# edin-dal/sdqlpy

Hardware: AMD Instinct MI355X
Metric: tpch_q1_q3_q5_sf10_rows_per_sec (higher is better)
Workload: dtype f64; 1 GPU; TPCH Q1+Q3+Q5 SF=10 per GPU (BASELINE metric: Q1/Q3/Q5 at SF=10; q1 = configs[1], q3 = configs[2]); partitioning=none

## Files before the change

### sdqlpy_amd/csrc/sdqh_hip.hip

```cpp
#include <hip/hip_runtime.h>

#include <algorithm>
#include <atomic>
#include <chrono>
#include <cmath>
#include <cstdio>
#include <cstdlib>
#include <cstring>
#include <string>
#include <thread>
#include <type_traits>
#include <map>
#include <vector>

#include "sdqh_host.hpp"

using namespace sdqh_host;

static int ensure_index(sdqh_ctx* ctx, sdqh_table* tb);

namespace sdqh_host {

int fail(sdqh_ctx* ctx, int code, const std::string& msg) {
    if (ctx) ctx->err = msg;
// ... 626 lines not shown
    else if (n == "delta8" && (value == 0 || value == 1)) ctx->opt_delta8 = (int)value;
    else if (n == "word_pairs" && (value == 0 || value == 1)) ctx->opt_word_pairs = (int)value;
    else if (n == "coarse_kb" && value >= 0 && value <= 96) ctx->opt_coarse_kb = (int)value;
    else if (n == "lookup_pipeline" && value >= -1 && value <= 1) ctx->opt_lookup_pipeline = (int)value;
    else if (n == "probe_pipeline" && value >= 0 && value <= 1) ctx->opt_probe_pipeline = (int)value;
    else if (n == "lookup_debug") ctx->opt_lookup_debug = (int)value;
    else if (n == "fuse_small" && value >= 0 && value <= 1) ctx->opt_fuse_small = (int)value;
    else if (n == "lds_key_set" && value >= 0 && value <= 1) ctx->opt_lds_key_set = (int)value;
    else if (n == "fill_ahead" && value >= 0 && value <= 1) { ctx->opt_fill_ahead = (int)value; for (auto& b : ctx->pool) b.nhabits = 0; }
    else if (n == "str_rows" && (value == 0 || value == 32 || value == 64)) ctx->opt_str_rows = (int)value;
    else if (n == "rank_increasing" && value >= 0 && value <= 1) ctx->opt_rank_increasing = (int)value;
    else if (n == "feature_min_rows" && value >= 0) ctx->opt_feature_min_rows = value;
    else if (n == "narrow" && value >= 0 && value <= 1) ctx->opt_narrow = (int)value;
    else if (n == "tight" && value >= 0 && value <= 1) ctx->opt_tight = (int)value;
    else if (n == "spin_sync" && value >= 0 && value <= 1) ctx->opt_spin_sync = (int)value;
    else if (n == "vstage" && value >= 0 && value <= 1) ctx->opt_vstage = (int)value;
    else if (n == "side_streams" && value >= 0 && value <= 1) ctx->opt_side_streams = (int)value;
    else if (n == "side_priority" && value >= 0 && value <= 1) ctx->opt_side_priority = (int)value;
    else if (n == "copy_kernel" && value >= 0 && value <= 4096) ctx->opt_copy_kernel = (int)value;
    else if (n == "copy_nt" && value >= 0 && value <= 1) ctx->opt_copy_nt = (int)value;
    else if (n == "x_waves" && value >= 0 && value <= 256) ctx->opt_x_waves = (int)value;
    else if (n == "window" && value >= 0 && value <= 1) ctx->opt_window = (int)value;
    else if (n == "lane_int" && value >= 0 && value <= 1) ctx->opt_lane_int = (int)value;
    else if (n == "row_index" && value >= 0 && value <= 1) ctx->opt_row_index = (int)value;
    else if (n == "lane_resident" && value >= 1 && value <= 4) ctx->opt_lane_resident = (int)value;
    else if (n == "async_result" && value >= 0 && value <= 1) ctx->opt_async_result = (int)value;
    else if (n == "stage_pipeline" && value >= 0 && value <= 1) ctx->opt_stage_pipeline = (int)value;
    else if (n == "span_index" && value >= 0 && value <= 1) ctx->opt_span_index = (int)value;
    else if (n == "dense_increasing" && value >= 0 && value <= 1) ctx->opt_dense_increasing = (int)value;
    else if (n == "packed_slots" && (value == 0 || value == 1)) ctx->opt_packed_slots = (int)value;
    else if (n == "grouped_index" && (value == 0 || value == 1)) ctx->opt_grouped_index = (int)value;
    else if (n == "grouped_pairs" && (value == 0 || value == 1)) ctx->opt_grouped_pairs = (int)value;
    else if (n == "index_inline" && (value == 0 || value == 1)) ctx->opt_index_inline = (int)value;
    else if (n == "groupby_regs" && (value == 0 || value == 4 || value == 8)) ctx->opt_groupby_regs = (int)value;
    else if (n == "hash_filter" && (value == 0 || value == 1)) ctx->opt_hash_filter = (int)value;
    else if (n == "pack_ordered" && (value == 0 || value == 1)) ctx->opt_pack_ordered = (int)value;
    else if (n == "pool_trim" && value == 1) {
        if (ctx->compile_only) return SDQH_OK;
        if (ctx->capturing) return fail(ctx, SDQH_ERR_UNSUPPORTED, "set_option: pool_trim inside a recording");
        (void)hipSetDevice(ctx->device);
        if (hipStreamSynchronize(ctx->stream) != hipSuccess) { (void)hipGetLastError(); return fail(ctx, SDQH_ERR_DEVICE, "pool_trim: the stream failed"); }
        for (auto& b : ctx->pool) if (b.free && b.ptr && !b.graph_owner) { (void)hipFree(b.ptr); b.ptr = nullptr; }
        ctx->pool.erase(std::remove_if(ctx->pool.begin(), ctx->pool.end(), [](const PoolBlock& b) { return b.ptr == nullptr; }), ctx->pool.end());
    }
    else return fail(ctx, SDQH_ERR_INVALID, "set_option: unknown option or value out of range: " + n);
    return SDQH_OK;
}

int sdqh_memory_stats(sdqh_ctx* ctx, int64_t* out, int n) {
    if (!ctx || !out || n < 4) return fail(ctx, SDQH_ERR_INVALID, "memory_stats: bad arguments");
    int64_t used = 0, cached = 0, graphs = 0, blocks = 0;
    for (const auto& b : ctx->pool) {
        if (!b.ptr) continue;
        ++blocks;
        if (b.graph_owner) graphs += (int64_t)b.size;
        if (b.free && !b.graph_owner) cached += (int64_t)b.size; else used += (int64_t)b.size;
    }
    out[0] = used; out[1] = cached; out[2] = graphs; out[3] = blocks;
    return SDQH_OK;
}

static int new_column(sdqh_ctx* ctx, int64_t nrows, int dtype, int width, sdqh_column** out) {
    if (!ctx || !out || nrows < 0) return fail(ctx, SDQH_ERR_INVALID, "column: bad arguments");
    if (dtype != SDQH_I64 && dtype != SDQH_F64 && dtype != SDQH_STR) return fail(ctx, SDQH_ERR_INVALID, "column: bad dtype");
    if (dtype == SDQH_STR && width < 1) return fail(ctx, SDQH_ERR_INVALID, "column: STR needs width >= 1");
    sdqh_column* c = new sdqh_column();
// ... 1272 lines not shown
        if (want_bm && ctx->opt_direct_index) { tb->nwords = lin_rb ? (lin_bits + 31) / 32 : ((uint64_t)(hi - lo) + 32) / 32; tb->bm = static_cast<uint32_t*>(table_alloc(ctx, tb, tb->nwords * 4 + 64)); }
        if (!tb->hdr || !flags || (tb->nwords && !tb->bm)) rc = fail(ctx, SDQH_ERR_NOMEM, "build: out of device memory");
    }
    uint32_t* grp_first = nullptr;
    const size_t grp_cells = grouped ? (size_t)(hi - lo) + 1 : 0;
    if (!rc && grouped && tb->bm) grp_first = static_cast<uint32_t*>(table_alloc(ctx, tb, grp_cells * 4 + 64));
    if (!rc) {
        tb->dev.hdr = tb->hdr; tb->dev.shits = tb->stage.shits; tb->dev.sacc = tb->stage.sacc; tb->dev.acc_stride = tb->stage.acc_stride;
        if (grp_first) {
            tb->stage.grp_first = grp_first;
            tb->dev.grp_first = grp_first; tb->dev.grp_key = tb->stage.key; tb->dev.grp_kstride = 1; tb->dev.grp_seg_rows = tb->stage.seg_rows;
            if (npayload >= 1 && ctx->opt_grouped_pairs) {
                int64_t* kp = static_cast<int64_t*>(table_alloc(ctx, tb, ((size_t)nrows + 8) * 16 + 64));
                if (kp) { tb->stage.grp_kp = kp; tb->dev.grp_key = kp; tb->dev.grp_kstride = 2; }
            } tb->dev.grp_cap = nrows + 1;
        }
        const int shift = (nkey == 2 && !(tb->bm && lin_rb)) ? 32 : 0;
        tb->dev.bm = tb->bm; tb->dev.bm_lo = lo; tb->dev.bm_hi = hi; tb->dev.bitmap_only = 0; tb->dev.bm_shift = shift;
        for (int p = 0; p < npayload; ++p) tb->dev.pay[p] = tb->stage.pay[p];
        tb->stage.bm = tb->bm; tb->stage.bm_lo = lo; tb->stage.bm_hi = hi; tb->stage.hdr = tb->hdr; tb->stage.bm_shift = shift;
        if (tb->bm && lin_rb) { tb->dev.lin_rb = tb->stage.lin_rb = lin_rb; tb->dev.lin_b0 = tb->stage.lin_b0 = lin_b0; }
        const unsigned seg_grid = (unsigned)((tb->stage.nseg + TPB / WAVE - 1) / (TPB / WAVE));
        FillList fl; fl.add(tb->hdr, sizeof(TableHeader), 0); fl.add(flags, 8, 0); if (tb->bm) fl.add(tb->bm, tb->nwords * 4, 0); prefill_refs(ctx, tb, &fl);
        if (grp_first) fl.add(grp_first, grp_cells * 4, 0xFF);
        DevFill pre; std::memset(&pre, 0, sizeof(pre));
        prune_clean(ctx, &fl);
        if (seg_grid == 1 && ctx->opt_fuse_small && fl.most <= ((uint64_t)1 << 20) && fl.f.n <= FILL_MAX) pre = fl.pre(); else launch_fill(ctx, fl);
        DevIndexInline ix; std::memset(&ix, 0, sizeof(ix));
        if (seg_grid == 1 && ctx->opt_fuse_small && ctx->opt_index_inline && tb->bm && shift == 0 && tb->refs_prefilled && (tb->nwords + RANK_BLOCK_WORDS - 1) / RANK_BLOCK_WORDS == 1) {
            uint32_t* wprefix = static_cast<uint32_t*>(table_alloc(ctx, tb, tb->nwords * 4 + 64));
            if (wprefix) {
                tb->dev.wprefix = wprefix;
                ix.t = tb->dev; ix.wprefix = wprefix; ix.span = tb->span; ix.nwords = tb->nwords; ix.on = 1;
            }
        }
        hipError_t e;
        with_scan_filter(f, [&](auto FC) {
            using FCT = decltype(FC);
            if constexpr (std::is_same_v<FCT, FCfg<1, 0, 0, 0>> || std::is_same_v<FCT, FCfg<0, 0, 0, 0>>) {
                const bool eager0 = nlookups > 0 && lookups[0].key[0].kind == SDQH_SRC_COLUMN && lookups[0].key[0].col->dtype == SDQH_I64;
                if (ctx->opt_narrow && nrows >= ctx->opt_feature_min_rows && (eager0 || f.ni == 1)) {
                    const int32_t* nkey0 = eager0 ? static_cast<const int32_t*>(ensure_narrow(ctx, const_cast<sdqh_column*>(lookups[0].key[0].col))) : nullptr;
                    const int32_t* npred0 = f.ni == 1 ? static_cast<const int32_t*>(ensure_narrow(ctx, const_cast<sdqh_column*>(filter->ipred[0].col))) : nullptr;
                    if ((!eager0 || nkey0) && (f.ni != 1 || npred0)) {
                        auto kern = k_build_lookup<FCT, true>;
                        LAUNCH(ctx, "k_build_lookup", kern, seg_grid, f, L, spec, tb->stage, nrows, flags, nkey0, npred0, pre, ix);
                        return SDQH_OK;
                    }
                }
            }
            auto kern = k_build_lookup<FCT>;
            LAUNCH(ctx, "k_build_lookup", kern, seg_grid, f, L, spec, tb->stage, nrows, flags, static_cast<const int32_t*>(nullptr), static_cast<const int32_t*>(nullptr), pre, ix);
            return SDQH_OK;
        });
        if (ix.on) { if (tb->span) tb->dev.dense_arr = tb->span; tb->index_built = true; }
        call_end(ctx);
        e = hipGetLastError();
        if (e != hipSuccess) rc = fail(ctx, SDQH_ERR_DEVICE, std::string("build launch: ") + hipGetErrorString(e));
        auto packs = [&](const sdqh_source& src) {
            if (src.kind != SDQH_SRC_COLUMN || !src.col || src.col->dtype != SDQH_I64) return false;
            sdqh_column* c = const_cast<sdqh_column*>(src.col);
            return ensure_minmax(ctx, c) == SDQH_OK && c->nrows > 0 && c->mn >= 0 && c->mx <= 0xFFFFFFFFll;
        };
        bool proven = composite;
        if (composite && !rc) {
            if (nkey == 2) proven = proven && packs(key[0]) && packs(key[1]);
            for (int l = 0; l < nlookups && proven; ++l) if (lookups[l].nkey == 2) proven = packs(lookups[l].key[0]) && packs(lookups[l].key[1]);
        }
        if (!rc && composite && !proven) {
            e = hipMemcpyAsync(ctx->result_host, flags, 4, hipMemcpyDeviceToHost, ctx->stream);
            if (e != hipSuccess) rc = fail(ctx, SDQH_ERR_DEVICE, hipGetErrorString(e));
            if (!rc) rc = sync_stream(ctx);
            if (!rc && (*static_cast<const int*>(ctx->result_host) & 2)) rc = fail(ctx, SDQH_ERR_UNSUPPORTED, "build: composite key part outside [0, 2^32)");
        }
    }
    if (rc) { table_release(ctx, tb); delete tb; return rc; }
    *out = tb;
    return SDQH_OK;
}

static int lookup_aggregate_launch(sdqh_ctx* ctx, int64_t nrows, const sdqh_filter* filter, int nlookups, const sdqh_lookup* lookups,
                                   int nkeys, const sdqh_source* keys, int tuple_shape, const sdqh_source* operands, void* block, bool device_block) {
    (void)hipSetDevice(ctx->device);
    const int nops = tuple_nops(tuple_shape), nv = tuple_nv(tuple_shape);
    if (nops < 0) return fail(ctx, SDQH_ERR_UNSUPPORTED, "unknown tuple shape");
// ... 556 lines not shown
```

### sdqlpy_amd/csrc/sdqh_host.hpp

```cpp
#pragma once
#include <hip/hip_runtime.h>

#include <atomic>
#include <map>
#include <string>
#include <vector>

#include "sdqh.h"
#include "sdqh_kernels.hpp"

namespace sdqh_host {

struct FillHabit { size_t off, bytes; int byte; bool clean; };
struct PoolBlock {
    void* ptr; size_t size; bool free;
    FillHabit habits[4] = {};
    int nhabits = 0;
    uint64_t alloc_seq = 0;
    bool fill_use = false;
    const void* graph_owner = nullptr;
};
struct ProfEntry { const char* name; hipEvent_t e0, e1; double ms; int64_t model_bytes; };

constexpr size_t STAGING_BYTES = 32u << 20;
// ... 43 lines not shown
    int opt_probe_chunk = 1;
    int opt_resident_stream = 2;
    int opt_probe_unroll = PROBE_UNROLL;
    int opt_stage_batch = STAGE_BATCH;
    int opt_stage_eager = 1;
    int nested = 0;
    int opt_stage_eager_pay = 0;
    int opt_stage_waves_per_cu = 12;
    int opt_direct_index = 1;
    int opt_packed_slots = 1;
    int opt_lookup_pipeline = -1;
    int opt_lookup_debug = 0;
    size_t rd_clean_ff = 0; int64_t rd_clean_zero_off = -1;
    int opt_fill_ahead = 1;
    uint64_t launch_seq = 0;
    int opt_lds_key_set = 1;
    int opt_fuse_small = 1;
    int opt_str_rows = 0;
    int opt_rank_increasing = 1;
    int64_t opt_feature_min_rows = 1 << 20;
    bool in_groupby_key = false;
    int opt_vstage = 1;
    int opt_tight = 1;
    hipStream_t side[2] = {nullptr, nullptr};
    hipEvent_t side_ev[4] = {nullptr, nullptr, nullptr, nullptr};
    int opt_side_streams = 1;
    int opt_side_priority = 1;
    int opt_copy_kernel = 0;
    int opt_copy_nt = 1;
    int opt_row_index = 1;
    int opt_grouped_index = 1;
    int opt_grouped_pairs = 1;
    int opt_index_inline = 1;
    int opt_lane_int = 1;
    int opt_lane_resident = 2;
    int opt_window = 0;
    int opt_x_driven = 64;
    int opt_word_pairs = 0;
    int opt_delta8 = 1;
    int opt_x_waves = 0;
    void* rs_dev[2] = {nullptr, nullptr}; size_t rs_bytes[2] = {0, 0};
    hipEvent_t rs_copied[2] = {nullptr, nullptr}; bool rs_used[2] = {false, false};
    int rs_cur = 0; bool rs_pending = false;
    hipEvent_t rs_ready = nullptr;
    volatile uint32_t* sync_flag = nullptr; uint32_t sync_seq = 0; int opt_spin_sync = 1;
    int opt_async_result = 1;
    int opt_narrow = 1;
    int opt_stage_pipeline = 0;
    int opt_span_index = 1;
    int opt_dense_increasing = 1;
    int opt_probe_pipeline = 0;
    const void* coarse_stat_col = nullptr; uint64_t* coarse_stat = nullptr;
    unsigned long long* coarse_count_dev = nullptr; uint64_t coarse_stat_bits_pending = 0; int coarse_skipped = 0; int64_t coarse_stat_build_rows = -1;
    int opt_coarse_kb = 64;
    int opt_row_pack = 1;
    struct RowPack { std::vector<const void*> cols; int64_t nrows; int k; void* data; const void* order_col = nullptr; void* key32 = nullptr;
                     void* lb = nullptr; int64_t key_lo = 0, key_hi = -1; };
    std::vector<RowPack> packs;
    int opt_pack_ordered = 1;
    int opt_hash_filter = 1;
    int opt_cluster_list = 1;
    int opt_cluster_pack = 1;
    int opt_groupby_regs = 0;
    const void* g4_hint[SDQH_MAX_GROUPKEYS] = {nullptr, nullptr};
};

// ... 136 lines not shown
```

### sdqlpy_amd/csrc/sdqh_kernels.hpp

```cpp
#pragma once
#ifndef __HIPCC_RTC__
#include <hip/hip_runtime.h>
#include <stdint.h>
#endif
#include "sdqh.h"

#if defined(__HIPCC_RTC__) || defined(SDQH_DECLS_ONLY)
#define SDQH_KERNEL template <int SDQH_RTC_UNUSED = 0> __global__
#else
#define SDQH_KERNEL __global__
#endif

namespace sdqh {

constexpr int TPB = 256;
constexpr int WAVE = 64;
constexpr int ROWS_PER_LOAD = 2;
#ifndef SDQH_UNROLL
#define SDQH_UNROLL 2
#endif
#ifndef SDQH_NT_LOADS
#define SDQH_NT_LOADS 1
#endif
#ifndef SDQH_TILE_CHUNK
// ... 63 lines not shown
    const int64_t* grp_key;
    int64_t grp_kstride;
    int64_t grp_seg_rows, grp_cap;
    const unsigned long long* wpair;
    uint32_t* hf;
};
constexpr int HF_SHIFT = 2;
constexpr uint32_t HF_POS_MASK = 0x07FFFFFFu;
constexpr uint64_t HF_MAX_CAP = 1ull << 22;
constexpr uint32_t HF_DEGENERATE = 127u;
__device__ __forceinline__ uint32_t hf_mask_of(uint64_t cap_mask) { return cap_mask + 1 > HF_MAX_CAP ? HF_DEGENERATE : (uint32_t)(((cap_mask + 1) << HF_SHIFT) - 1); }
__device__ __forceinline__ uint32_t hf_raw(int64_t key);
__device__ __forceinline__ uint32_t hf_code(uint32_t raw, uint32_t mask) { return (raw & mask) | (raw & ~HF_POS_MASK); }
__device__ __forceinline__ uint32_t hf_bits(uint32_t code) { return (1u << (code & 31u)) | (1u << (code >> 27)); }
__device__ __forceinline__ bool hf_test(uint32_t word, uint32_t code) { return ((word >> (code & 31u)) & (word >> (code >> 27)) & 1u) != 0u; }

constexpr int FILL_MAX = 6;
struct DevFill { void* p[FILL_MAX]; uint64_t bytes[FILL_MAX]; uint32_t word[FILL_MAX]; int32_t n, _pad; };
constexpr int FILL_BIG = 32;
struct DevFillBig { void* p[FILL_BIG]; uint64_t bytes[FILL_BIG]; uint32_t word[FILL_BIG]; int32_t n, _pad; };
__device__ __forceinline__ void fill_in_block(const DevFill& f) {
#pragma unroll
    for (int r = 0; r < FILL_MAX; ++r) {
        if (r >= f.n) break;
        const uint32_t w = f.word[r];
        const uint64_t n16 = f.bytes[r] / 16, n4 = f.bytes[r] / 4;
        uint4* p16 = static_cast<uint4*>(f.p[r]);
        for (uint64_t i = threadIdx.x; i < n16; i += blockDim.x) p16[i] = make_uint4(w, w, w, w);
        uint32_t* p4 = static_cast<uint32_t*>(f.p[r]);
        for (uint64_t i = n16 * 4 + threadIdx.x; i < n4; i += blockDim.x) p4[i] = w;
    }
}

__device__ __forceinline__ int64_t slot_key(const DevTable& t, uint64_t h) { return t.slots ? t.slots[h * 4] : t.keys[h]; }
__device__ __forceinline__ uint32_t slot_row(const DevTable& t, uint64_t h) { return t.slots ? (uint32_t)t.slots[h * 4 + 3] : t.rowref[h]; }

template <class T>
__device__ __forceinline__ bool bm_locate(const T& t, int64_t key, uint64_t& off) {
    const int64_t rb = t.lin_rb;
    const int64_t v = (t.bm_shift || rb) ? (int64_t)((uint64_t)key >> 32) : key;
    if (v < t.bm_lo || v > t.bm_hi) return false;
    off = (uint64_t)(v - t.bm_lo);
    if (rb) {
        const int64_t b = (int64_t)((uint64_t)key & 0xFFFFFFFFull) - t.lin_b0;
        if (b < 0 || b >= rb) return false;
        off = off * (uint64_t)rb + (uint64_t)b;
    }
    return true;
}

template <int SHAPE> struct TupleTraits;
template <> struct TupleTraits<SDQH_TUPLE_A>          { static constexpr int NOPS = 1, NV = 1; };
template <> struct TupleTraits<SDQH_TUPLE_AB>         { static constexpr int NOPS = 2, NV = 1; };
template <> struct TupleTraits<SDQH_TUPLE_A_1MB>      { static constexpr int NOPS = 2, NV = 1; };
template <> struct TupleTraits<SDQH_TUPLE_PRICING>    { static constexpr int NOPS = 4, NV = 4; };
template <> struct TupleTraits<SDQH_TUPLE_A_1MB_M_CD> { static constexpr int NOPS = 4, NV = 1; };
template <> struct TupleTraits<SDQH_TUPLE_COUNT>      { static constexpr int NOPS = 0, NV = 0; };

template <int SHAPE>
__device__ __forceinline__ void tuple_eval(const double (&x)[4], double (&o)[4]) {
    if constexpr (SHAPE == SDQH_TUPLE_A) { o[0] = x[0]; }
    else if constexpr (SHAPE == SDQH_TUPLE_AB) { o[0] = x[0] * x[1]; }
    else if constexpr (SHAPE == SDQH_TUPLE_A_1MB) { o[0] = x[0] * (1.0 - x[1]); }
    else if constexpr (SHAPE == SDQH_TUPLE_PRICING) {
        double dp = x[1] * (1.0 - x[2]);
        o[0] = x[0]; o[1] = x[1]; o[2] = dp; o[3] = dp * (1.0 + x[3]);
// ... 1236 lines not shown
    }
    int t = s - 1;
    while (t > 0 && st.seg_count[t] == 0) --t;
    WordExc e;
    e.key0 = f.key; e.pos0 = f.pos; e.n0 = n_below; e._pad = 0;
    e.pos_prev = (uint32_t)((int64_t)t * st.seg_rows + (int64_t)st.seg_count[t] - (int64_t)n_below);
    exc[s] = e;
    st.wrow[w0] = ROW_INDEX_EXC | (uint32_t)s;
}
__device__ __forceinline__ bool direct_has_dups(const TableHeader* hdr) { return hdr->staged != hdr->distinct; }
SDQH_KERNEL __launch_bounds__(TPB) void k_fill_refs(DevStage st, DevTable t) {
    if (!direct_has_dups(t.hdr)) return;
    const uint64_t n = t.hdr->distinct;
    for (uint64_t i = (uint64_t)blockIdx.x * TPB + threadIdx.x; i < n; i += (uint64_t)gridDim.x * TPB) t.dense_ref[i] = NO_ROW;
}
__device__ __forceinline__ void insert_direct_body(const DevStage& st, const DevTable& t, uint32_t* __restrict__ span) {
    const int seg = blockIdx.x * (TPB / WAVE) + threadIdx.x / WAVE;
    const bool dups = direct_has_dups(t.hdr);
    if (blockIdx.x == 0 && threadIdx.x == 0) t.hdr->has_dups = dups ? 1u : 0u;
    if (seg >= st.nseg) return;
    const int64_t base = (int64_t)seg * st.seg_rows;
    const uint32_t count = st.seg_count[seg];
    for (uint32_t i = lane_id(); i < count; i += WAVE) {
        const int64_t idx = base + i;
        const int64_t pos = table_find(t, st.key[idx], 0);
        if (pos < 0) continue;
        if (dups) atomicMin(&t.dense_ref[pos], (uint32_t)idx); else t.dense_ref[pos] = (uint32_t)idx;
        if (span) { uint32_t* cell = span + (st.key[idx] - t.bm_lo); if (dups) atomicMin(cell, (uint32_t)idx); else *cell = (uint32_t)idx; }
    }
}
SDQH_KERNEL __launch_bounds__(TPB) void k_insert_direct(DevStage st, DevTable t, uint32_t* __restrict__ span) { insert_direct_body(st, t, span); }
SDQH_KERNEL __launch_bounds__(TPB) void k_index_small(const uint32_t* __restrict__ bm, uint64_t nwords, uint32_t* __restrict__ wprefix, DevStage st, DevTable t, uint32_t* __restrict__ span) {
    rank_words_body(bm, nwords, wprefix, st.seg_count, st.nseg, t.hdr);
    __threadfence();
    __syncthreads();
    insert_direct_body(st, t, span);
}
SDQH_KERNEL __launch_bounds__(TPB) void k_index_medium(const uint32_t* __restrict__ bm, uint32_t nwords, uint32_t* __restrict__ wprefix, DevStage st, DevTable t, uint32_t* __restrict__ span) {
    __shared__ uint32_t s_word[RANK_BLOCK_WORDS], s_pre[RANK_BLOCK_WORDS];
    __shared__ uint32_t s_wave[TPB / WAVE];
    __shared__ uint32_t s_staged;
    constexpr int PER = RANK_BLOCK_WORDS / TPB;
    const int lane = lane_id(), w = threadIdx.x / WAVE;
    for (int i = threadIdx.x; i < RANK_BLOCK_WORDS; i += TPB) s_word[i] = (uint32_t)i < nwords ? bm[i] : 0u;
    if (threadIdx.x == 0) s_staged = 0u;
    __syncthreads();
    uint32_t mine = 0;
#pragma unroll
    for (int j = 0; j < PER; ++j) mine += (uint32_t)__popc(s_word[threadIdx.x * PER + j]);
    uint32_t incl = mine;
#pragma unroll
    for (int off = 1; off < WAVE; off <<= 1) { const uint32_t v = __shfl_up(incl, off, WAVE); if (lane >= off) incl += v; }
    if (lane == WAVE - 1) s_wave[w] = incl;
    uint32_t stg = 0;
    for (int i = threadIdx.x; i < st.nseg; i += TPB) stg += st.seg_count[i];
#pragma unroll
    for (int off = WAVE / 2; off > 0; off >>= 1) stg += __shfl_down(stg, off, WAVE);
    if (lane == 0 && stg) atomicAdd(&s_staged, stg);
    __syncthreads();
    uint32_t before = 0, total = 0;
#pragma unroll
    for (int i = 0; i < TPB / WAVE; ++i) { if (i < w) before += s_wave[i]; total += s_wave[i]; }
    uint32_t run = before + incl - mine;
#pragma unroll
    for (int j = 0; j < PER; ++j) { s_pre[threadIdx.x * PER + j] = run; run += (uint32_t)__popc(s_word[threadIdx.x * PER + j]); }
    __syncthreads();
    const uint32_t staged = s_staged;
    const bool dups = staged != total;
// ... 757 lines not shown
    if (!t.bm) return true;
    if (L.l[0].nkey == 2 && t.bm_shift == 0) return true;
    if (part0 < t.bm_lo || part0 > t.bm_hi) return false;
    const uint64_t off = (uint64_t)(part0 - t.bm_lo);
    return (t.bm[off >> 5] >> (off & 31)) & 1u;
}

__device__ __forceinline__ bool first_lookup_none(const DevLookups& L) {
    const DevTable& t = L.l[0].table;
    return !t.bm || (L.l[0].nkey == 2 && t.bm_shift == 0);
}
__device__ __forceinline__ uint32_t first_lookup_word(const DevLookups& L, int64_t part0) {
    const DevTable& t = L.l[0].table;
    const bool in = part0 >= t.bm_lo && part0 <= t.bm_hi;
    const uint64_t off = in ? (uint64_t)(part0 - t.bm_lo) : 0;
    return t.bm[off >> 5];
}
__device__ __forceinline__ bool first_lookup_bit(const DevLookups& L, int64_t part0, uint32_t word) {
    const DevTable& t = L.l[0].table;
    const bool in = part0 >= t.bm_lo && part0 <= t.bm_hi;
    return in && ((word >> ((uint64_t)(part0 - t.bm_lo) & 31)) & 1u);
}

constexpr int BUILD_LB = 4;
constexpr int LOOKUP_PU = 2;
constexpr int LBQ_CAP = 64 + BUILD_LB * 128;

struct DevBuildSpec {
    int32_t nkey, npay;
    DevSource key[2];
    DevSource pay[SDQH_MAX_PAYLOAD];
};

struct DevIndexInline { DevTable t; uint32_t* wprefix; uint32_t* span; uint64_t nwords; int32_t on, _pad; };

template <class FC, bool NW>
__device__ __forceinline__ void build_lookup_segment(const DevFilter& f, const DevLookups& L, const DevBuildSpec& spec, const DevStage& st, int64_t nrows, int* __restrict__ flags,
                                                     const int32_t* __restrict__ nkey0, const int32_t* __restrict__ npred0, int32_t* q_row, const int seg) {
    const int64_t* skey0 = NW ? reinterpret_cast<const int64_t*>(nkey0) : L.l[0].key[0].col;
    const int64_t begin = (int64_t)seg * st.seg_rows;
    int64_t end = begin + st.seg_rows; if (end > nrows) end = nrows;
    const int lane = lane_id();
    const uint64_t lt = lanemask_lt();
    constexpr int64_t BATCH_ROWS = WAVE * ROWS_PER_LOAD;
    const bool eager0 = L.n > 0 && L.l[0].key[0].kind == SDQH_SRC_COLUMN;
    DevProbes none; none.n = 0;
    const uint64_t nomask[SDQH_MAX_PROBE] = {0, 0};
    int64_t out = begin;
    int qn = 0;
    bool bad = false;
    auto drain = [&](int first, int count) {
        bool keep = false; int64_t key = 0; int64_t pay[MAX_STAGE_COLS] = {0, 0, 0, 0, 0};
        if (lane < count) {
            const int64_t r = begin + (int64_t)q_row[first + lane];
            uint32_t ent[SDQH_MAX_LOOKUP] = {0, 0, 0};
            const PackRow nopack{};
            const int h = run_lookups(L, r, ent, nopack);
            if (h < 0) bad = true;
            if (h > 0) {
                const int64_t p0 = source_value(spec.key[0], L, r, ent, nopack);
                const int64_t p1 = spec.nkey == 2 ? source_value(spec.key[1], L, r, ent, nopack) : 0;
                if (pack_parts(spec.nkey, p0, p1, key)) bad = true;
                else {
                    keep = true;
#pragma unroll
                    for (int q = 0; q < SDQH_MAX_PAYLOAD; ++q) if (q < spec.npay) pay[q] = source_value(spec.pay[q], L, r, ent, nopack);
                }
// ... 59 lines not shown
            enqueue(r, p1b[0][0], p1b[0][1]);
            b += BATCH_ROWS;
        }
        int head = 0;
        while (qn - head >= WAVE || (last && qn > head)) {
            const int n = qn - head >= WAVE ? WAVE : qn - head;
            drain(head, n);
            head += n;
        }
        if (last) break;
        if (head) {
            const int left = qn - head;
            int32_t keepv = 0;
            if (lane < left) keepv = q_row[head + lane];
            if (lane < left) q_row[lane] = keepv;
            qn = left;
        }
    }
    if (lane == 0) {
        st.seg_count[seg] = (uint32_t)(out - begin);
        stage_end_segment(st, seg, begin, out - begin);
        if (st.grp_first && seg == 0) st.hdr->has_dups = 1u;
    }
    if (__ballot(bad) && lane == 0) atomicOr(flags, 2);
}

template <class FC, bool NW = false>
__global__ __launch_bounds__(TPB) void k_build_lookup(DevFilter f, DevLookups L, DevBuildSpec spec, DevStage st, int64_t nrows, int* __restrict__ flags,
                                                      const int32_t* __restrict__ nkey0, const int32_t* __restrict__ npred0, DevFill pre, DevIndexInline ix) {
    if (pre.n) { fill_in_block(pre); __syncthreads(); }
    __shared__ int32_t s_row[TPB / WAVE][LBQ_CAP];
    const int seg = blockIdx.x * (TPB / WAVE) + threadIdx.x / WAVE;
    if (seg < st.nseg) build_lookup_segment<FC, NW>(f, L, spec, st, nrows, flags, nkey0, npred0, s_row[threadIdx.x / WAVE], seg);
    if (ix.on) {
        __threadfence();
        __syncthreads();
        rank_words_body(st.bm, ix.nwords, ix.wprefix, st.seg_count, st.nseg, st.hdr);
        __threadfence();
        __syncthreads();
        insert_direct_body(st, ix.t, ix.span);
    }
}

struct DevPackCols { const int64_t* col[MAX_PACK]; int32_t ncols, k; };
SDQH_KERNEL __launch_bounds__(TPB) void k_interleave(DevPackCols c, int64_t nrows, int64_t* __restrict__ out) {
    for (int64_t r = (int64_t)blockIdx.x * TPB + threadIdx.x; r < nrows; r += (int64_t)gridDim.x * TPB) {
        int64_t v[MAX_PACK];
#pragma unroll
        for (int j = 0; j < MAX_PACK; ++j) v[j] = j < c.ncols ? c.col[j][r] : 0;
#pragma unroll
        for (int j = 0; j < MAX_PACK; ++j) if (j < c.k) out[r * c.k + j] = v[j];
    }
}

constexpr int LG_SLOTS = 2 * SDQH_MAX_LOOKUP_GROUPS;

struct DevAggSpec {
    int32_t nkeys, shape;
    DevSource key[SDQH_MAX_GROUPKEYS];
    DevSource op[4];
};

__device__ __forceinline__ int group_slot(unsigned long long* keys, unsigned long long key, bool global) {
    int h = (int)(mix64(key) & (LG_SLOTS - 1));
#pragma unroll 1
    for (int i = 0; i < LG_SLOTS; ++i) {
        unsigned long long cur = global ? __hip_atomic_load(&keys[h], __ATOMIC_RELAXED, __HIP_MEMORY_SCOPE_AGENT) : keys[h];
        if (cur == EMPTY_GROUP) cur = atomicCAS(&keys[h], (unsigned long long)EMPTY_GROUP, key);
        if (cur == EMPTY_GROUP || cur == key) return h;
        h = (h + 1) & (LG_SLOTS - 1);
    }
    return -1;
}
// ... 769 lines not shown
```

### sdqlpy_amd/csrc/sdqh_x.hip

```cpp
#define SDQH_DECLS_ONLY 1
#include <hip/hip_runtime.h>
#include <hip/hiprtc.h>

#include <dlfcn.h>
#include <sys/stat.h>
#include <unistd.h>

#include <algorithm>
#include <chrono>
#include <cstdio>
#include <cstdlib>
#include <cstring>
#include <fstream>
#include <mutex>
#include <sstream>
#include <string>
#include <vector>

#include "sdqh_host.hpp"
#include "sdqh_xkernels.hpp"

using namespace sdqh_host;

namespace {
// ... 1134 lines not shown
    }
    if (const char* env = std::getenv("SDQLPY_AMD_JIT_CACHE")) J.cache_dir = env;
    else J.cache_dir = dir + "/../jit_cache";
    (void)mkdir(J.cache_dir.c_str(), 0777);
    return true;
}

uint64_t structure_hash(const XInfo& x, Sink sink, bool direct) {
    const sdqh_program* p = x.p;
    uint64_t h = 1469598103934665603ull;
    auto mix = [&](uint64_t v) { h ^= v; h *= 0x9E3779B97F4A7C15ull; h ^= h >> 29; };
    mix((uint64_t)sink * 2 + (direct ? 1 : 0)); mix((uint64_t)x.narrow_mask);
    if (x.tight) {
        mix(0x7167ull); mix((uint64_t)x.gather32); mix((x.pref32 ? 1ull : 0ull) | (x.vstage ? 2ull : 0ull) | (x.pwin ? 4ull : 0ull) | (x.pnear ? 8ull : 0ull) | (x.driven ? 16ull : 0ull) | (x.phash ? 32ull : 0ull) | ((uint64_t)(x.ival + 1) << 8));
        for (int c = 0; c < x.ncols; ++c) mix(((uint64_t)(uint32_t)x.enc[c] << 32) | ((uint32_t)(x.affine[c] ? 1 : 0) << 16) | (uint32_t)(x.dict_slot[c] & 0xFFFF));
        for (int k = 0; k < x.p->nops; ++k) mix((uint64_t)(uint8_t)x.irange[k]);
        for (int k = 0; k < x.p->nops; ++k) mix(((uint64_t)(uint32_t)x.cmp_cc[k] << 32) | ((uint32_t)x.cmp_kind[k] << 8) | (uint32_t)(x.cmp_col[k] & 0xFF));
    } mix((uint64_t)p->nops); mix((uint64_t)(int64_t)p->key); mix((uint64_t)(int64_t)x.probe_op);
    for (int k = 0; k < p->nops; ++k) {
        const sdqh_xop& o = p->ops[k];
        mix(((uint64_t)(uint32_t)o.code << 32) | (uint32_t)o.type); mix(((uint64_t)(uint32_t)o.a << 32) | (uint32_t)o.b); mix(((uint64_t)(uint32_t)o.c << 32) | (uint32_t)o.aux);
        mix(((uint64_t)(uint32_t)x.col_of[k] << 32) | (uint32_t)x.tab_of[k]); mix(((uint64_t)(uint32_t)x.const_of[k] << 32) | (uint32_t)x.str_off[k]);
        if (o.code == SDQH_X_DIVI || o.code == SDQH_X_MODI) mix((uint64_t)o.imm_i);
        if (o.code == SDQH_X_STR || o.code == SDQH_X_STRIDX) { mix((uint64_t)o.slen); for (int i = 0; i < o.slen; ++i) mix(o.str[i]); }
        if (o.code == SDQH_X_STR || o.code == SDQH_X_STRIDX || o.code == SDQH_X_CHAR) mix((uint64_t)(o.col ? o.col->width : 0));
    }
    mix((uint64_t)p->ngates); for (int g = 0; g < p->ngates; ++g) mix((uint64_t)p->gates[g]);
    mix((uint64_t)p->nvals); for (int v = 0; v < p->nvals; ++v) mix((uint64_t)p->vals[v]);
    return h;
}

int specialise(sdqh_ctx* ctx, const std::string& source, const std::string& entry, hipFunction_t* fn);

int kernel_for(sdqh_ctx* ctx, const XInfo& x, Sink sink, bool direct, hipFunction_t* fn) {
    JitState& J = jit();
    static const bool no_layouts = std::getenv("SDQLPY_AMD_X_NOLAYOUT") != nullptr;
    uint64_t lay_hash = 0;
    for (int t = 0; t < x.ntabs; ++t) {
        if (ctx->compile_only) { x.lay[t] = 0u; continue; }
        if (int rc = index_ensure(ctx, x.tabs[t])) return rc;
        x.lay[t] = no_layouts ? 0u : x_layout_of(x.tabs[t]->dev, x.tabs[t]->bitmap_only);
        lay_hash = (lay_hash ^ x.lay[t]) * 0x9E3779B97F4A7C15ull + (uint64_t)t;
    }
    char name[64];
    std::snprintf(name, sizeof(name), "s%016llx@%d", (unsigned long long)(structure_hash(x, sink, direct) ^ lay_hash), ctx->device);
    if (!ctx->compile_only) {
        std::lock_guard<std::mutex> lock(J.mu);
        auto hit = J.kernels.find(name);
        if (hit != J.kernels.end()) { *fn = hit->second; return SDQH_OK; }
    }
    if (int rc = specialise(ctx, generate(x, sink, direct), (x.vstage && sink == SINK_STAGE) ? std::string(VSTAGE_ENTRY) : entry_name(sink, direct, x.tight), fn)) return rc;
    std::lock_guard<std::mutex> lock(J.mu);
    J.kernels[name] = *fn;
    return SDQH_OK;
}

int specialise(sdqh_ctx* ctx, const std::string& source_in, const std::string& entry, hipFunction_t* fn) {
    std::string source = source_in;
    if (const char* defs = std::getenv("SDQLPY_AMD_X_DEFINES")) {
        std::istringstream in(defs); std::string tok, head;
        while (in >> tok) { const size_t eq = tok.find('='); head += "#define " + (eq == std::string::npos ? tok + " 1" : tok.substr(0, eq) + " " + tok.substr(eq + 1)) + "\n"; }
        source = head + source;
    }
    JitState& J = jit();
    std::lock_guard<std::mutex> lock(J.mu);
    if (!load_headers(J)) return fail(ctx, SDQH_ERR_DEVICE, J.why_unusable);
    int rtc_major = 0, rtc_minor = 0;
    (void)hiprtcVersion(&rtc_major, &rtc_minor);
    uint64_t h = fnv1a(source);
    h = fnv1a(J.h_xkernels, h); h = fnv1a(J.h_kernels, h); h = fnv1a(J.h_abi, h);
    h = fnv1a("gfx950 rtc " + std::to_string(rtc_major) + "." + std::to_string(rtc_minor), h);
    char name[64];
// ... 22 lines not shown
            return fail(ctx, SDQH_ERR_DEVICE, std::string("hiprtc: ") + hiprtcGetErrorString(r) + "\n" + log.substr(0, 4000));
        }
        size_t n = 0; (void)hiprtcGetCodeSize(prog, &n);
        code.resize(n);
        (void)hiprtcGetCode(prog, &code[0]);
        (void)hiprtcDestroyProgram(&prog);
        ++J.compiled;
        if (const char* rdir = std::getenv("SDQLPY_AMD_JIT_RECIPES")) {
            char rn[32]; std::snprintf(rn, sizeof(rn), "%016llx", (unsigned long long)fnv1a(source));
            (void)mkdir(rdir, 0777);
            std::ofstream rf(std::string(rdir) + "/" + rn + ".hip", std::ios::binary);
            rf << source;
        }
        const std::string tmp = path + ".tmp." + std::to_string((long)getpid());
        { std::ofstream f(tmp, std::ios::binary); f.write(code.data(), (std::streamsize)code.size()); }
        (void)std::rename(tmp.c_str(), path.c_str());
    }
    if (ctx->compile_only) return fail(ctx, SDQH_ERR_DEVICE, "compile-only context: kernel specialised (" + std::to_string(code.size()) + " bytes of gfx950 code), not run");
    hipModule_t mod;
    if (hipModuleLoadData(&mod, code.data()) != hipSuccess) { (void)hipGetLastError(); return fail(ctx, SDQH_ERR_DEVICE, "hipModuleLoadData failed for a specialised kernel"); }
    hipFunction_t f;
    if (hipModuleGetFunction(&f, mod, entry.c_str()) != hipSuccess) { (void)hipGetLastError(); return fail(ctx, SDQH_ERR_DEVICE, "specialised kernel has no entry point"); }
    J.kernels[key] = f;
    *fn = f;
    return SDQH_OK;
}

template <class SA> struct Packed { XArgs a; SA s; int64_t nrows; int64_t seg_rows; int32_t nseg; };

int fill_xargs(sdqh_ctx* ctx, const XInfo& x, XArgs* a, int32_t* flags, int64_t key_lo, int64_t key_hi) {
    std::memset(a, 0, sizeof(*a));
    for (int c = 0; c < x.ncols; ++c) { a->col[c] = x.cols[c]->data; a->width[c] = x.cols[c]->width; a->ncol[c] = (((x.narrow_mask | x.gather32) >> c) & 1u) ? x.cols[c]->narrow : nullptr; }
    for (int t = 0; t < x.ntabs; ++t) {
        if (int rc = index_ensure(ctx, x.tabs[t])) return rc;
        a->tab[t] = x.tabs[t]->dev;
    }
    if (x.tight) for (int c = 0; c < x.ncols; ++c) a->dlo[c] = x.dlo[c];
    if (x.tight) for (int c = 0; c < x.ncols; ++c) if (x.enc[c] == ENC_D8) a->dcol[c] = x.cols[c]->delta8;
    if (x.tight) for (int c = 0; c < x.ncols; ++c) if (x.enc[c] >= ENC_C16) { a->code[c] = x.cols[c]->code; a->dict[c] = static_cast<const int64_t*>(x.cols[c]->dict); a->ndict[c] = x.cols[c]->ndict; }
    std::memcpy(a->cc, x.cc, sizeof(x.cc[0]) * (size_t)x.ncc);
    std::memcpy(a->ci, x.ci, sizeof(x.ci[0]) * (size_t)x.nci);
    std::memcpy(a->cf, x.cf, sizeof(x.cf[0]) * (size_t)x.ncf);
    std::memcpy(a->spool, x.spool, sizeof(uint32_t) * (size_t)x.nstr);
    a->flags = flags; a->key_lo = key_lo; a->key_hi = key_hi;
    if (x.driven && x.driven_col >= 0 && x.cols[x.driven_col]->run_index_state == 1) {
        const sdqh_column* kc = x.cols[x.driven_col];
        a->run_index = static_cast<const uint32_t*>(kc->run_index); a->run_lo = kc->mn; a->run_hi = kc->mx; a->driven_ratio = ctx->opt_x_driven;
    }
    return SDQH_OK;
}

struct Geometry { unsigned grid; int64_t seg_rows; int nseg; };
Geometry geometry_tight(sdqh_ctx* ctx, int64_t nrows, int resident, bool pipelined = false) {
    const int64_t steps = std::max<int64_t>(1, nrows / ((int64_t)XT_ROWS * (pipelined ? 1 : 2)));
    return Geometry{(unsigned)std::min<int64_t>(steps, (int64_t)ctx->num_cu * resident), 0, 0};
}
Geometry geometry(sdqh_ctx* ctx, int64_t nrows, bool direct, int waves_per_cu, bool tight = false, bool tiled = false) {
    Geometry g{1, 0, 0};
    static const bool no_tiles = getenv("SDQLPY_AMD_X_NOTILED") != nullptr;
    if (tiled && tight && !direct && !no_tiles && nrows < ((int64_t)1 << 31) && nrows >= (int64_t)X8_STEP * X8_U) {
        if (ctx->opt_x_waves > 0) waves_per_cu = ctx->opt_x_waves;
        const int64_t steps = nrows / ((int64_t)X8_STEP * X8_U);
        g.seg_rows = 0;
        g.nseg = (int)std::max<int64_t>(1, std::min<int64_t>(steps, (int64_t)ctx->num_cu * waves_per_cu));
        g.grid = (unsigned)((g.nseg + TPB / WAVE - 1) / (TPB / WAVE));
        return g;
    }
// ... 541 lines not shown
```

Measured before the change: 451.2 billion rows/s.

## Skip index build for membership-only probe tables and speed inline indexing

Adds a member_bits option so that probe tables used only for membership tests in fused kernels are treated as bitmap-only, which skips building their dense row index. The inline index step inside k_build_lookup is replaced with a single-block shared-memory rank and insert, with LDS sized at launch. The fence and sync sequence is also swapped for a waitcnt-plus-scoped-fence handover. The risk lies in the layout hash and correctness when a table is later used for field access, since its index may then be built lazily.

Measured after the change: 451.0 billion rows/s, median of 2. Within noise of the previous version (-0.0%).

```diff
diff --git a/sdqlpy_amd/csrc/sdqh_hip.hip b/sdqlpy_amd/csrc/sdqh_hip.hip
--- a/sdqlpy_amd/csrc/sdqh_hip.hip
+++ b/sdqlpy_amd/csrc/sdqh_hip.hip
@@ -682,6 +682,7 @@
     else if (n == "grouped_index" && (value == 0 || value == 1)) ctx->opt_grouped_index = (int)value;
     else if (n == "grouped_pairs" && (value == 0 || value == 1)) ctx->opt_grouped_pairs = (int)value;
     else if (n == "index_inline" && (value == 0 || value == 1)) ctx->opt_index_inline = (int)value;
+    else if (n == "member_bits" && (value == 0 || value == 1)) ctx->opt_member_bits = (int)value;
     else if (n == "groupby_regs" && (value == 0 || value == 4 || value == 8)) ctx->opt_groupby_regs = (int)value;
     else if (n == "hash_filter" && (value == 0 || value == 1)) ctx->opt_hash_filter = (int)value;
     else if (n == "pack_ordered" && (value == 0 || value == 1)) ctx->opt_pack_ordered = (int)value;
@@ -2020,8 +2021,10 @@
             if (wprefix) {
                 tb->dev.wprefix = wprefix;
                 ix.t = tb->dev; ix.wprefix = wprefix; ix.span = tb->span; ix.nwords = tb->nwords; ix.on = 1;
+                ix.per = (int32_t)std::max<uint64_t>(1, (tb->nwords + TPB - 1) / TPB);
             }
         }
+        const size_t ix_lds = ix.on ? (size_t)ix.per * TPB * 2 * sizeof(uint32_t) : 0;
         hipError_t e;
         with_scan_filter(f, [&](auto FC) {
             using FCT = decltype(FC);
@@ -2032,13 +2035,13 @@
                     const int32_t* npred0 = f.ni == 1 ? static_cast<const int32_t*>(ensure_narrow(ctx, const_cast<sdqh_column*>(filter->ipred[0].col))) : nullptr;
                     if ((!eager0 || nkey0) && (f.ni != 1 || npred0)) {
                         auto kern = k_build_lookup<FCT, true>;
-                        LAUNCH(ctx, "k_build_lookup", kern, seg_grid, f, L, spec, tb->stage, nrows, flags, nkey0, npred0, pre, ix);
+                        LAUNCH_LDS(ctx, "k_build_lookup", kern, seg_grid, ix_lds, f, L, spec, tb->stage, nrows, flags, nkey0, npred0, pre, ix);
                         return SDQH_OK;
                     }
                 }
             }
             auto kern = k_build_lookup<FCT>;
-            LAUNCH(ctx, "k_build_lookup", kern, seg_grid, f, L, spec, tb->stage, nrows, flags, static_cast<const int32_t*>(nullptr), static_cast<const int32_t*>(nullptr), pre, ix);
+            LAUNCH_LDS(ctx, "k_build_lookup", kern, seg_grid, ix_lds, f, L, spec, tb->stage, nrows, flags, static_cast<const int32_t*>(nullptr), static_cast<const int32_t*>(nullptr), pre, ix);
             return SDQH_OK;
         });
         if (ix.on) { if (tb->span) tb->dev.dense_arr = tb->span; tb->index_built = true; }
diff --git a/sdqlpy_amd/csrc/sdqh_host.hpp b/sdqlpy_amd/csrc/sdqh_host.hpp
--- a/sdqlpy_amd/csrc/sdqh_host.hpp
+++ b/sdqlpy_amd/csrc/sdqh_host.hpp
@@ -99,6 +99,7 @@
     int opt_grouped_index = 1;
     int opt_grouped_pairs = 1;
     int opt_index_inline = 1;
+    int opt_member_bits = 1;
     int opt_lane_int = 1;
     int opt_lane_resident = 2;
     int opt_window = 0;
diff --git a/sdqlpy_amd/csrc/sdqh_kernels.hpp b/sdqlpy_amd/csrc/sdqh_kernels.hpp
--- a/sdqlpy_amd/csrc/sdqh_kernels.hpp
+++ b/sdqlpy_amd/csrc/sdqh_kernels.hpp
@@ -119,6 +119,15 @@
     }
 }
 
+__device__ __forceinline__ void block_handover() {
+#if defined(__HIP_DEVICE_COMPILE__)
+    __builtin_amdgcn_s_waitcnt(0);
+    __builtin_amdgcn_fence(__ATOMIC_RELEASE, "workgroup");
+    __syncthreads();
+    __builtin_amdgcn_fence(__ATOMIC_ACQUIRE, "agent");
+#endif
+}
+
 __device__ __forceinline__ int64_t slot_key(const DevTable& t, uint64_t h) { return t.slots ? t.slots[h * 4] : t.keys[h]; }
 __device__ __forceinline__ uint32_t slot_row(const DevTable& t, uint64_t h) { return t.slots ? (uint32_t)t.slots[h * 4 + 3] : t.rowref[h]; }
 
@@ -1421,8 +1430,7 @@
 SDQH_KERNEL __launch_bounds__(TPB) void k_insert_direct(DevStage st, DevTable t, uint32_t* __restrict__ span) { insert_direct_body(st, t, span); }
 SDQH_KERNEL __launch_bounds__(TPB) void k_index_small(const uint32_t* __restrict__ bm, uint64_t nwords, uint32_t* __restrict__ wprefix, DevStage st, DevTable t, uint32_t* __restrict__ span) {
     rank_words_body(bm, nwords, wprefix, st.seg_count, st.nseg, t.hdr);
-    __threadfence();
-    __syncthreads();
+    block_handover();
     insert_direct_body(st, t, span);
 }
 SDQH_KERNEL __launch_bounds__(TPB) void k_index_medium(const uint32_t* __restrict__ bm, uint32_t nwords, uint32_t* __restrict__ wprefix, DevStage st, DevTable t, uint32_t* __restrict__ span) {
@@ -2246,7 +2254,50 @@
     DevSource pay[SDQH_MAX_PAYLOAD];
 };
 
-struct DevIndexInline { DevTable t; uint32_t* wprefix; uint32_t* span; uint64_t nwords; int32_t on, _pad; };
+struct DevIndexInline { DevTable t; uint32_t* wprefix; uint32_t* span; uint64_t nwords; int32_t on, per; };
+
+__device__ __forceinline__ void index_solo_body(const DevStage& st, const DevTable& t, uint32_t* __restrict__ wprefix, uint32_t* __restrict__ span, uint32_t nwords,
+                                                uint32_t* s_word, uint32_t* s_pre, int per) {
+    __shared__ uint32_t s_wave[TPB / WAVE];
+    __shared__ uint32_t s_staged;
+    const int lane = lane_id(), w = threadIdx.x / WAVE;
+    const uint32_t cap = (uint32_t)per * TPB;
+    for (uint32_t i = threadIdx.x; i < cap; i += TPB) s_word[i] = i < nwords ? st.bm[i] : 0u;
+    const uint32_t count = w < st.nseg ? st.seg_count[w] : 0u;
+    if (threadIdx.x == 0) s_staged = 0u;
+    __syncthreads();
+    uint32_t mine = 0;
+    for (int j = 0; j < per; ++j) mine += (uint32_t)__popc(s_word[threadIdx.x * per + j]);
+    uint32_t incl = mine;
+#pragma unroll
+    for (int off = 1; off < WAVE; off <<= 1) { const uint32_t v = __shfl_up(incl, off, WAVE); if (lane >= off) incl += v; }
+    if (lane == WAVE - 1) s_wave[w] = incl;
+    if (lane == 0 && count) atomicAdd(&s_staged, count);
+    __syncthreads();
+    uint32_t before = 0, total = 0;
+#pragma unroll
+    for (int i = 0; i < TPB / WAVE; ++i) { if (i < w) before += s_wave[i]; total += s_wave[i]; }
+    uint32_t run = before + incl - mine;
+    for (int j = 0; j < per; ++j) { s_pre[threadIdx.x * per + j] = run; run += (uint32_t)__popc(s_word[threadIdx.x * per + j]); }
+    __syncthreads();
+    const uint32_t staged = s_staged;
+    const bool dups = staged != total;
+    for (uint32_t i = threadIdx.x; i < nwords; i += TPB) wprefix[i] = s_pre[i];
+    if (threadIdx.x == 0) { t.hdr->staged = staged; t.hdr->distinct = total; t.hdr->has_dups = dups ? 1u : 0u; }
+    if (w >= st.nseg) return;
+    const int64_t base = (int64_t)w * st.seg_rows;
+    for (uint32_t i = lane; i < count; i += WAVE) {
+        const int64_t idx = base + i;
+        const int64_t key = st.key[idx];
+        uint64_t off;
+        if (!bm_locate(t, key, off) || (off >> 5) >= (uint64_t)nwords) continue;
+        const uint32_t word = s_word[off >> 5];
+        if (!((word >> (off & 31)) & 1u)) continue;
+        const uint32_t pos = s_pre[off >> 5] + (uint32_t)__popc(word & ((1u << (off & 31)) - 1u));
+        if (dups) atomicMin(&t.dense_ref[pos], (uint32_t)idx); else t.dense_ref[pos] = (uint32_t)idx;
+        if (span) { uint32_t* cell = span + (key - t.bm_lo); if (dups) atomicMin(cell, (uint32_t)idx); else *cell = (uint32_t)idx; }
+    }
+}
 
 template <class FC, bool NW>
 __device__ __forceinline__ void build_lookup_segment(const DevFilter& f, const DevLookups& L, const DevBuildSpec& spec, const DevStage& st, int64_t nrows, int* __restrict__ flags,
@@ -2372,13 +2423,10 @@
     __shared__ int32_t s_row[TPB / WAVE][LBQ_CAP];
     const int seg = blockIdx.x * (TPB / WAVE) + threadIdx.x / WAVE;
     if (seg < st.nseg) build_lookup_segment<FC, NW>(f, L, spec, st, nrows, flags, nkey0, npred0, s_row[threadIdx.x / WAVE], seg);
+    extern __shared__ __align__(16) uint32_t s_ix[];
     if (ix.on) {
-        __threadfence();
-        __syncthreads();
-        rank_words_body(st.bm, ix.nwords, ix.wprefix, st.seg_count, st.nseg, st.hdr);
-        __threadfence();
-        __syncthreads();
-        insert_direct_body(st, ix.t, ix.span);
+        block_handover();
+        index_solo_body(st, ix.t, ix.wprefix, ix.span, (uint32_t)ix.nwords, s_ix, s_ix + (size_t)ix.per * TPB, ix.per);
     }
 }
 
diff --git a/sdqlpy_amd/csrc/sdqh_x.hip b/sdqlpy_amd/csrc/sdqh_x.hip
--- a/sdqlpy_amd/csrc/sdqh_x.hip
+++ b/sdqlpy_amd/csrc/sdqh_x.hip
@@ -1190,12 +1190,32 @@
 
 int specialise(sdqh_ctx* ctx, const std::string& source, const std::string& entry, hipFunction_t* fn);
 
+static bool x_no_layouts() { static const bool v = std::getenv("SDQLPY_AMD_X_NOLAYOUT") != nullptr; return v; }
+
+static bool x_membership_only(const sdqh_ctx* ctx, const XInfo& x, int t) {
+    const sdqh_table* tb = x.tabs[t];
+    if (!ctx->opt_member_bits || x_no_layouts() || tb->index_built || tb->bitmap_only) return false;
+    const DevTable& d = tb->dev;
+    if (!d.bm || d.bm_shift != 0 || d.grp_first || d.dense_arr || d.alias) return false;
+    if (x.probe_op >= 0 && x.tab_of[x.probe_op] == t) return false;
+    for (int k = 0; k < x.p->nops; ++k) {
+        const sdqh_xop& o = x.p->ops[k];
+        if ((o.code == SDQH_X_FIELD || o.code == SDQH_X_ACC) && x.tab_of[o.a] == t) return false;
+    }
+    return true;
+}
+
 int kernel_for(sdqh_ctx* ctx, const XInfo& x, Sink sink, bool direct, hipFunction_t* fn) {
     JitState& J = jit();
-    static const bool no_layouts = std::getenv("SDQLPY_AMD_X_NOLAYOUT") != nullptr;
+    const bool no_layouts = x_no_layouts();
     uint64_t lay_hash = 0;
     for (int t = 0; t < x.ntabs; ++t) {
         if (ctx->compile_only) { x.lay[t] = 0u; continue; }
+        if (x_membership_only(ctx, x, t)) {
+            x.lay[t] = x_layout_of(x.tabs[t]->dev, true);
+            lay_hash = (lay_hash ^ x.lay[t]) * 0x9E3779B97F4A7C15ull + (uint64_t)t;
+            continue;
+        }
         if (int rc = index_ensure(ctx, x.tabs[t])) return rc;
         x.lay[t] = no_layouts ? 0u : x_layout_of(x.tabs[t]->dev, x.tabs[t]->bitmap_only);
         lay_hash = (lay_hash ^ x.lay[t]) * 0x9E3779B97F4A7C15ull + (uint64_t)t;
@@ -1284,7 +1304,7 @@
     std::memset(a, 0, sizeof(*a));
     for (int c = 0; c < x.ncols; ++c) { a->col[c] = x.cols[c]->data; a->width[c] = x.cols[c]->width; a->ncol[c] = (((x.narrow_mask | x.gather32) >> c) & 1u) ? x.cols[c]->narrow : nullptr; }
     for (int t = 0; t < x.ntabs; ++t) {
-        if (int rc = index_ensure(ctx, x.tabs[t])) return rc;
+        if (!x_membership_only(ctx, x, t)) if (int rc = index_ensure(ctx, x.tabs[t])) return rc;
         a->tab[t] = x.tabs[t]->dev;
     }
     if (x.tight) for (int c = 0; c < x.ncols; ++c) a->dlo[c] = x.dlo[c];
diff --git a/sdqlpy_amd/jit_recipes/73dcef449c700af5.hip b/sdqlpy_amd/jit_recipes/73dcef449c700af5.hip
--- /dev/null
+++ b/sdqlpy_amd/jit_recipes/73dcef449c700af5.hip
@@ -0,0 +1,54 @@
+#include "sdqh_xkernels.hpp"
+using namespace sdqh;
+struct P {
+    static constexpr int NS = 1, NV = 1, NSC = 0, NSOP = 0, ND = 0;
+    struct Regs { uint32_t c0[16]; };
+    __device__ __forceinline__ static void load_dicts(const XArgs& a, int64_t (*tab)[256]) {
+    }
+    template <bool TAIL> __device__ __forceinline__ static void sload(const XArgs& a, int64_t r, int64_t nrows, Regs& s) {
+        xt_load<8, TAIL>(a.col[0], r, nrows, s.c0);
+    }
+    __device__ __forceinline__ static bool stest(const XArgs& a, const Regs& s, const int64_t (*tab)[256], const int i) {
+        bool p = true;
+        const int64_t v0 = xt_i64(s.c0, i);
+        p = p && x_may_hit(a.tab[0], v0, false);
+        return p;
+    }
+    __device__ __forceinline__ static bool spre(const XArgs& a, const Regs& s, const int64_t (*tab)[256], const int i, uint32_t& widx, uint32_t& bit) {
+        bool p = true;
+        const int64_t v0 = xt_i64(s.c0, i);
+        const bool in = (v0 >= a.tab[0].bm_lo) & (v0 <= a.tab[0].bm_hi);
+        p = p & in;
+        const uint64_t off = p ? (uint64_t)(v0 - a.tab[0].bm_lo) : 0ull;
+        widx = (uint32_t)(off >> 5); bit = (uint32_t)off & 31u;
+        return p;
+    }
+    static constexpr bool PREF32 = false, PWIN = false;
+    __device__ __forceinline__ static bool spre32(const XArgs& a, const Regs& s, const int64_t (*tab)[256], const int i, uint32_t& off) {
+        off = 0; return false;
+    }
+    __device__ __forceinline__ static const uint32_t* sbitmap(const XArgs& a) { return x_prefilter_bitmap(a.tab[0], false); }
+    template <int H> __device__ __forceinline__ static bool eval_regs(const XArgs& a, const Pair<int64_t> (&s)[1], int64_t r, XOut<NV>& o) {
+        return false;
+    }
+    __device__ __forceinline__ static bool eval_row(const XArgs& a, int64_t r, const int64_t (&sres)[1], XOut<NV>& o) {
+        int64_t v0 = static_cast<const int64_t*>(a.col[0])[r];
+        x_pin(v0);
+        const uint32_t e1 = x_lookup_l<0x8000004au>(a.tab[0], v0, false);
+        const bool v1 = (e1 != NO_ROW);
+        if (!v1) return false;
+        double v2 = static_cast<const double*>(a.col[1])[r];
+        double v3 = static_cast<const double*>(a.col[2])[r];
+        x_pin(v2, v3);
+        o.key = 0; o.bad = false;
+        const double v4 = (v2 * v3);
+        const double v5 = a.cf[0];
+        const double v6 = (v4 * v5);
+        o.val[0] = x_bits(v6);
+        o.ent = NO_ROW;
+        return true;
+    }
+};
+extern "C" __global__ __launch_bounds__(256) void xk_sum_tight(XArgs a, XSum<P::NV>::Args s, int64_t nrows, int64_t seg_rows, int nseg) {
+    x_queue8<P, XSum, false>(a, s, nrows, seg_rows, nseg);
+}
diff --git a/sdqlpy_amd/jit_recipes/87af1fbbadc4f9dd.hip b/sdqlpy_amd/jit_recipes/87af1fbbadc4f9dd.hip
--- /dev/null
+++ b/sdqlpy_amd/jit_recipes/87af1fbbadc4f9dd.hip
@@ -0,0 +1,71 @@
+#include "sdqh_xkernels.hpp"
+using namespace sdqh;
+struct P {
+    static constexpr int NS = 1, NV = 1, NSC = 0, NSOP = 0, ND = 0;
+    struct Regs { uint32_t c0[8]; };
+    __device__ __forceinline__ static void load_dicts(const XArgs& a, int64_t (*tab)[256]) {
+    }
+    template <bool TAIL> __device__ __forceinline__ static void sload(const XArgs& a, int64_t r, int64_t nrows, Regs& s) {
+        xt_load<4, TAIL>(a.ncol[0], r, nrows, s.c0);
+    }
+    __device__ __forceinline__ static bool stest(const XArgs& a, const Regs& s, const int64_t (*tab)[256], const int i) {
+        bool p = true;
+        const int64_t v0 = (int64_t)xt_i32(s.c0, i);
+        p = p && x_may_hit(a.tab[0], v0, false);
+        return p;
+    }
+    __device__ __forceinline__ static bool spre(const XArgs& a, const Regs& s, const int64_t (*tab)[256], const int i, uint32_t& widx, uint32_t& bit) {
+        bool p = true;
+        const int64_t v0 = (int64_t)xt_i32(s.c0, i);
+        const bool in = (v0 >= a.tab[0].bm_lo) & (v0 <= a.tab[0].bm_hi);
+        p = p & in;
+        const uint64_t off = in ? (uint64_t)(v0 - a.tab[0].bm_lo) : 0ull;
+        widx = (uint32_t)(off >> 5); bit = (uint32_t)off & 31u;
+        return p;
+    }
+    static constexpr bool PREF32 = true, PWIN = false;
+    __device__ __forceinline__ static bool spre32(const XArgs& a, const Regs& s, const int64_t (*tab)[256], const int i, uint32_t& off) {
+        bool p = true;
+        const int64_t v0 = (int64_t)xt_i32(s.c0, i);
+        const uint32_t o32 = (uint32_t)((int32_t)v0 - (int32_t)a.tab[0].bm_lo);
+        const bool in = o32 <= (uint32_t)(a.tab[0].bm_hi - a.tab[0].bm_lo);
+        p = p & in;
+        off = in ? o32 : 0u;
+        return p;
+    }
+    __device__ __forceinline__ static const uint32_t* sbitmap(const XArgs& a) { return x_prefilter_bitmap(a.tab[0], false); }
+    static constexpr bool DRIVEN = true;
+    __device__ __forceinline__ static const DevTable& dtab(const XArgs& a) { return a.tab[0]; }
+    template <int H> __device__ __forceinline__ static bool eval_regs(const XArgs& a, const Pair<int64_t> (&s)[1], int64_t r, XOut<NV>& o) {
+        return false;
+    }
+    __device__ __forceinline__ static bool eval_row(const XArgs& a, int64_t r, const int64_t (&sres)[1], XOut<NV>& o) {
+        int64_t v0 = (int64_t)static_cast<const int32_t*>(a.ncol[0])[r];
+        int64_t v2 = (int64_t)static_cast<const int32_t*>(a.ncol[1])[r];
+        x_pin(v0, v2);
+        const uint32_t e1 = x_lookup_l<0x80000082u>(a.tab[0], v0, false);
+        const bool v1 = (e1 != NO_ROW);
+        int64_t v3 = x_field(a.tab[0], 1, e1);
+        x_pin(v3);
+        if (!v1) return false;
+        const bool b4 = false || false || v2 < 0 || v2 > 0xFFFFFFFFll || v3 < 0 || v3 > 0xFFFFFFFFll;
+        const int64_t v4 = (int64_t)(((uint64_t)v2 << 32) | ((uint64_t)v3 & 0xFFFFFFFFull));
+        const uint32_t e5 = x_lookup_l<0x8000005au>(a.tab[1], v4, b4);
+        const bool v5 = (e5 != NO_ROW);
+        if (!v5) return false;
+        int64_t v6 = x_field(a.tab[0], 0, e1);
+        double v7 = narrow_decode(static_cast<const int32_t*>(a.ncol[2])[r]);
+        double v9 = narrow_decode(static_cast<const int32_t*>(a.ncol[3])[r]);
+        x_pin(v6, v7, v9);
+        o.key = v6; o.bad = false;
+        const double v8 = a.cf[0];
+        const double v10 = (v8 - v9);
+        const double v11 = (v7 * v10);
+        o.val[0] = x_bits(v11);
+        o.ent = NO_ROW;
+        return true;
+    }
+};
+extern "C" __global__ __launch_bounds__(256) void xk_group_tight(XArgs a, XGroup<P::NV>::Args s, int64_t nrows, int64_t seg_rows, int nseg) {
+    x_queue8<P, XGroup, false>(a, s, nrows, seg_rows, nseg);
+}
```
